# magicat777/Audio-Analyzer-OMEGA

Measured on NVIDIA B200. Metric: stream-seconds of 48 kHz stereo analysed/sec (multi-res FFT+LUFS+TP), higher is better.
Workload: dtype f32 (FFT, combine, K-weighting in a float32 delta-form state, sample peaks of the true-peak meter; its four transforms per frame pair in f16x2; tensor-core GEMM on (hi, lo) half operands with fp32 accumulators for the few-bin resolutions) + f64 (meter statistics)

## Files before the change

### audio-analyzer-omega_b200/csrc/kweight32_kernel.cuh

```cuda
#pragma once
#include <cuda_runtime.h>
#include "kweight_kernel.cuh"
#include "blockdft_tc_kernel.cuh"

namespace o4 {

struct Kw32Sec {
    float b0, a2, gamma, bb;
    float phi[5][4];
    float c16[4], c17[4];
    float g[KW_SUBMAX][2];
    float2 ga0[16], ga1[16];
};

struct Kweight32Args {
    const float* x;
    long long ch_stride, frame_stride, frame_off0;
    int n_ch, n_frames, first_frame, frames_per_warp;
    const float* hann;
    double* lufs_out;
    int rms_gate, _align;
    float* hop_inv;
    int hop_inv_nb, hop_inv_j0;
    Kw32Sec s[2];
};

__device__ __forceinline__ float2 kw32_mat(const float* m, float2 s) {
    return make_float2(fmaf(m[0], s.x, m[1] * s.y), fmaf(m[2], s.x, m[3] * s.y));
}

struct Kw32R { float r0; float2 a[16]; float2 b[16]; };

__device__ __forceinline__ float& kwr(Kw32R& q, int i) {
    if (i == 0) return q.r0;
    if (i <= 16) return q.a[i - 1].x;
    if (i <= 32) return q.b[i - 17].x;
    if (i <= 48) return q.b[i - 33].y;
    return q.a[i - 49].y;
}
__device__ __forceinline__ float2 bc2(float v) { return make_float2(v, v); }

template <bool BACKWARD>
__device__ __forceinline__ void kw32_pass(Kw32R& q, const Kw32Sec& c, int lane) {
    const int pos = BACKWARD ? 31 - lane : lane;
    const float b0 = c.b0, a2 = c.a2, ngamma = -c.gamma, bb = c.bb;
    float xa_in, dxa_in;
    {
        const float p1 = BACKWARD ? __shfl_down_sync(0xffffffffu, kwr(q, 0), 1) : __shfl_up_sync(0xffffffffu, kwr(q, KW_L - 1), 1);
        const float p2 = BACKWARD ? __shfl_down_sync(0xffffffffu, kwr(q, 1), 1) : __shfl_up_sync(0xffffffffu, kwr(q, KW_L - 2), 1);
        const float x0 = BACKWARD ? kwr(q, KW_L - 1) : kwr(q, 0);
        xa_in = pos == 0 ? x0 : p1;
        dxa_in = pos == 0 ? 0.f : p1 - p2;
    }
    const float2 s0 = make_float2(-b0 * xa_in, 0.f);
    float2 xaA, dxaA, xaB, dxaB;
    if (!BACKWARD) {
        xaA = make_float2(xa_in, kwr(q, 48)); dxaA = make_float2(dxa_in, kwr(q, 48) - kwr(q, 47));
        xaB = make_float2(kwr(q, 16), kwr(q, 32)); dxaB = make_float2(kwr(q, 16) - kwr(q, 15), kwr(q, 32) - kwr(q, 31));
    } else {
        xaA = make_float2(kwr(q, 17), xa_in); dxaA = make_float2(kwr(q, 17) - kwr(q, 18), dxa_in);
        xaB = make_float2(kwr(q, 33), kwr(q, 49)); dxaB = make_float2(kwr(q, 33) - kwr(q, 34), kwr(q, 49) - kwr(q, 50));
    }
    float2 zA = bc2(0.f), dA = bc2(0.f), yA = make_float2(b0 * xaA.x, b0 * xaA.y);
    float2 zB = bc2(0.f), dB = bc2(0.f), yB = make_float2(b0 * xaB.x, b0 * xaB.y);
    if (!BACKWARD) {
        const float x = q.r0;
        const float t = fmaf(a2, dA.x, dxaA.x);
        const float d = fmaf(ngamma, yA.x, t);
        const float z = fmaf(bb, d, zA.x);
        const float y = fmaf(b0, x, z);
        dxaA.x = x - xaA.x; xaA.x = x; zA.x = z; dA.x = d; yA.x = y;
        q.r0 = y;
    }
    const float2 A2 = bc2(a2), NG = bc2(ngamma), BB = bc2(bb), B0 = bc2(b0);
#pragma unroll
    for (int n = 0; n < 16; ++n) {
        const int k = BACKWARD ? 15 - n : n;
        {
            const float2 x = q.a[k];
            const float2 t = __ffma2_rn(A2, dA, dxaA);
            const float2 d = __ffma2_rn(NG, yA, t);
            const float2 z = __ffma2_rn(BB, d, zA);
            const float2 y = __ffma2_rn(B0, x, z);
            dxaA = __fadd2_rn(x, make_float2(-xaA.x, -xaA.y)); xaA = x; zA = z; dA = d; yA = y;
            q.a[k] = y;
        }
        {
            const float2 x = q.b[k];
            const float2 t = __ffma2_rn(A2, dB, dxaB);
            const float2 d = __ffma2_rn(NG, yB, t);
            const float2 z = __ffma2_rn(BB, d, zB);
            const float2 y = __ffma2_rn(B0, x, z);
            dxaB = __fadd2_rn(x, make_float2(-xaB.x, -xaB.y)); xaB = x; zB = z; dB = d; yB = y;
            q.b[k] = y;
        }
    }
    if (BACKWARD) {
        const float x = q.r0;
        const float t = fmaf(a2, dA.x, dxaA.x);
        const float d = fmaf(ngamma, yA.x, t);
        const float z = fmaf(bb, d, zA.x);
        const float y = fmaf(b0, x, z);
        zA.x = z; dA.x = d;
        q.r0 = y;
    }
    float2 e[KW_NSUB];
    if (!BACKWARD) { e[0] = make_float2(zA.x, dA.x); e[1] = make_float2(zB.x, dB.x); e[2] = make_float2(zB.y, dB.y); e[3] = make_float2(zA.y, dA.y); }
    else           { e[0] = make_float2(zA.y, dA.y); e[1] = make_float2(zB.y, dB.y); e[2] = make_float2(zB.x, dB.x); e[3] = make_float2(zA.x, dA.x); }
    float2 v = e[0];
#pragma unroll
    for (int m = 1; m < KW_NSUB; ++m) {
        const int j = BACKWARD ? KW_NSUB - 1 - m : m;
        const float* cm = (kw_off(j + 1) - kw_off(j) == 17) ? c.c17 : c.c16;
        const float2 w = kw32_mat(cm, v);
        v = make_float2(w.x + e[m].x, w.y + e[m].y);
    }
    if (pos == 0) {
        const float2 w = kw32_mat(c.phi[0], s0);
        v.x += w.x; v.y += w.y;
    }
#pragma unroll
    for (int jj = 0; jj < 5; ++jj) {
        const int dd = 1 << jj;
        const float rx = BACKWARD ? __shfl_down_sync(0xffffffffu, v.x, dd) : __shfl_up_sync(0xffffffffu, v.x, dd);
        const float ry = BACKWARD ? __shfl_down_sync(0xffffffffu, v.y, dd) : __shfl_up_sync(0xffffffffu, v.y, dd);
        if (pos >= dd) {
            const float2 w = kw32_mat(c.phi[jj], make_float2(rx, ry));
            v.x += w.x; v.y += w.y;
        }
    }
    float2 sin[KW_NSUB];
    sin[0].x = BACKWARD ? __shfl_down_sync(0xffffffffu, v.x, 1) : __shfl_up_sync(0xffffffffu, v.x, 1);
    sin[0].y = BACKWARD ? __shfl_down_sync(0xffffffffu, v.y, 1) : __shfl_up_sync(0xffffffffu, v.y, 1);
    if (pos == 0) sin[0] = s0;
#pragma unroll
    for (int m = 1; m < KW_NSUB; ++m) {
        const int jp = BACKWARD ? KW_NSUB - m : m - 1;
        const float* cm = (kw_off(jp + 1) - kw_off(jp) == 17) ? c.c17 : c.c16;
        const float2 w = kw32_mat(cm, sin[m - 1]);
        sin[m] = make_float2(w.x + e[m - 1].x, w.y + e[m - 1].y);
    }
    const float2 s_c0 = BACKWARD ? sin[3] : sin[0], s_c1 = BACKWARD ? sin[2] : sin[1];
    const float2 s_c2 = BACKWARD ? sin[1] : sin[2], s_c3 = BACKWARD ? sin[0] : sin[3];
    const float2 SXA = make_float2(s_c0.x, s_c3.x), SYA = make_float2(s_c0.y, s_c3.y);
    const float2 SXB = make_float2(s_c1.x, s_c2.x), SYB = make_float2(s_c1.y, s_c2.y);
    if (!BACKWARD) {
        q.r0 = fmaf(c.g[0][0], s_c0.x, fmaf(c.g[0][1], s_c0.y, q.r0));
#pragma unroll
        for (int k = 0; k < 16; ++k) {
            q.a[k] = __ffma2_rn(c.ga0[k], SXA, __ffma2_rn(c.ga1[k], SYA, q.a[k]));
            q.b[k] = __ffma2_rn(bc2(c.g[k][0]), SXB, __ffma2_rn(bc2(c.g[k][1]), SYB, q.b[k]));
        }
    } else {
#pragma unroll
        for (int k = 0; k < 16; ++k) {
            const float2 G0 = bc2(c.g[15 - k][0]), G1 = bc2(c.g[15 - k][1]);
            q.a[k] = __ffma2_rn(G0, SXA, __ffma2_rn(G1, SYA, q.a[k]));
            q.b[k] = __ffma2_rn(G0, SXB, __ffma2_rn(G1, SYB, q.b[k]));
        }
        q.r0 = fmaf(c.g[16][0], s_c0.x, fmaf(c.g[16][1], s_c0.y, q.r0));
    }
}

__device__ __forceinline__ void kw32_odd_pad(Kw32R& q, int lane) {
    if (lane == 0) {
#pragma unroll
        for (int j = 0; j < KW_PAD; ++j) kwr(q, j) = 2.f * kwr(q, KW_PAD) - kwr(q, 2 * KW_PAD - j);
    }
    if (lane == 31) {
        constexpr int E = KW_LAST - KW_PAD;
#pragma unroll
        for (int j = 0; j < KW_PAD; ++j) kwr(q, E + 1 + j) = 2.f * kwr(q, E) - kwr(q, E - 1 - j);
#pragma unroll
        for (int i = KW_LAST + 1; i < KW_L; ++i) kwr(q, i) = kwr(q, KW_LAST);
    }
}

__device__ __forceinline__ void kw32_fill_slack(Kw32R& q, int lane) {
    if (lane == 31) {
#pragma unroll
        for (int i = KW_LAST + 1; i < KW_L; ++i) kwr(q, i) = kwr(q, KW_LAST);
    }
}

__device__ __forceinline__ void kw32_zero_pads(Kw32R& q, int lane) {
    if (lane == 0) {
#pragma unroll
        for (int i = 0; i < KW_PAD; ++i) kwr(q, i) = 0.f;
    }
    if (lane == 31) {
#pragma unroll
        for (int i = KW_LAST - KW_PAD + 1; i < KW_L; ++i) kwr(q, i) = 0.f;
    }
}

constexpr int KW32_WARPS = 4;
#ifndef KW32_MIN_BLOCKS
#define KW32_MIN_BLOCKS 3
#endif

__global__ void __launch_bounds__(KW32_WARPS * 32, KW32_MIN_BLOCKS)
kweight32_kernel(const __grid_constant__ Kweight32Args a) {
    extern __shared__ __align__(16) unsigned char smem_raw[];
    float* hann_x = reinterpret_cast<float*>(smem_raw);
    float* stage_all = hann_x + 32 * KW_L;
    const int lane = threadIdx.x & 31;
    const int warp = threadIdx.x >> 5;
    float* stg = stage_all + warp * KW_STG;

    for (int p = threadIdx.x; p < 32 * KW_L; p += blockDim.x) {
        const int n = p - KW_PAD;
        hann_x[p] = (n >= 0 && n < KW_W) ? a.hann[n] : 0.f;
    }
    __syncthreads();

    const int frames_per_cta = a.frames_per_warp * KW32_WARPS;
    const int tiles_per_ch = (a.n_frames + frames_per_cta - 1) / frames_per_cta;
    const int ch = blockIdx.x / tiles_per_ch;
    const int tile = blockIdx.x % tiles_per_ch;

    for (int it = 0; it < a.frames_per_warp; ++it) {
        const int f = tile * frames_per_cta + it * KW32_WARPS + warp;
        if (f >= a.n_frames || f < a.first_frame) continue;
        const long long off = (long long)ch * a.ch_stride + a.frame_off0 + (long long)f * a.frame_stride;

        const float4* px = reinterpret_cast<const float4*>(a.x + off);
        float4* s4 = reinterpret_cast<float4*>(stg + KW_PAD + KW_STG_SHIFT);
        float4 tmp[KW_W / 4 / 32];
#pragma unroll
        for (int j = 0; j < KW_W / 4 / 32; ++j) tmp[j] = __ldg(px + lane + 32 * j);
        if (a.hop_inv) {
            float m = 0.f;
#pragma unroll
            for (int j = 3 * KW_W / 4 / 4 / 32; j < KW_W / 4 / 32; ++j)
                m = fmaxf(fmaxf(m, fmaxf(fabsf(tmp[j].x), fabsf(tmp[j].y))), fmaxf(fabsf(tmp[j].z), fabsf(tmp[j].w)));
#pragma unroll
            for (int o = 16; o > 0; o >>= 1) m = fmaxf(m, __shfl_xor_sync(0xffffffffu, m, o));
            if (lane == 0) a.hop_inv[(size_t)ch * a.hop_inv_nb + (f - a.hop_inv_j0)] = hop_row_scale(m);
        }
        if (lane < KW_PAD) stg[KW_STG_SHIFT + lane] = 0.f;
        if (lane < KW_SLACK + KW_PAD + KW_STG_SHIFT) stg[KW_STG_SHIFT + KW_PAD + KW_W + lane] = 0.f;
#pragma unroll
        for (int j = 0; j < KW_W / 4 / 32; ++j) s4[lane + 32 * j] = tmp[j];
        __syncwarp();
        float* sl = stg + KW_STG_SHIFT + KW_L * lane;
        const float* hl = hann_x + KW_L * lane;
        Kw32R r;
        float sumsq = 0.f;
#pragma unroll
        for (int i = 0; i < KW_L; ++i) {
            const float xv = sl[i] * hl[i];
            sumsq = fmaf(xv, xv, sumsq);
            kwr(r, i) = xv;
        }
        __syncwarp();
#pragma unroll
        for (int o = 16; o > 0; o >>= 1) sumsq += __shfl_xor_sync(0xffffffffu, sumsq, o);
        const bool gated = a.rms_gate && sqrtf(sumsq * (1.f / KW_W)) < 1e-6f;

        double ms = 0.0;
        if (!gated) {
#ifdef KW32_UNROLL_SECTIONS
#pragma unroll
#else
#pragma unroll 1
#endif
            for (int si = 0; si < 2; ++si) {
                const Kw32Sec& c = a.s[si];
                kw32_odd_pad(r, lane);
                kw32_pass<false>(r, c, lane);
                kw32_fill_slack(r, lane);
                kw32_pass<true>(r, c, lane);
                if (si == 0) {
                    kw32_zero_pads(r, lane);
#pragma unroll
                    for (int i = 0; i < KW_L; ++i) sl[i] = kwr(r, i);
                }
            }
            kw32_zero_pads(r, lane);
            float acc = 0.f;
#pragma unroll
            for (int i = 0; i < KW_L; ++i) {
                const float fv = sl[i];
                const float w = fmaf(kwr(r, i) - fv, 0.3f, fv);
                acc = fmaf(w, w, acc);
            }
#pragma unroll
            for (int o = 16; o > 0; o >>= 1) acc += __shfl_xor_sync(0xffffffffu, acc, o);
            ms = (double)acc / (double)KW_W;
            __syncwarp();
        }
        if (lane == 0)
            a.lufs_out[(size_t)ch * a.n_frames + f] = (ms > 1e-10) ? (-0.691 + 10.0 * log10(ms)) : -100.0;
    }
}

inline size_t kweight32_smem_bytes() {
    return (size_t)32 * KW_L * sizeof(float) + (size_t)KW32_WARPS * KW_STG * sizeof(float);
}

}
```

### audio-analyzer-omega_b200/csrc/omega4_cuda.cu

```cuda
#include "../../include/omega4_cuda.h"

#include <cuda_runtime.h>
#include <math.h>
#include <stdio.h>
#include <stdlib.h>
#include <string.h>

#include <algorithm>
#include <map>
#include <mutex>
#include <set>
#include <string>
#include <vector>

#include "bars_kernel.cuh"
#include "blockdft_kernel.cuh"
#include "blockdft_tc_kernel.cuh"
#include "fft_core.cuh"
#include "kweight_kernel.cuh"
#include "kweight32_kernel.cuh"
#include "loudness_kernel.cuh"
#include "misc_kernels.cuh"
#include "octave_kernel.cuh"
#include "multires_kernel.cuh"
// ... 155 lines not shown

static int launch_kweight(const KweightArgs& a, cudaStream_t s) {
    if (a.x_is_f64) return a.weighted_out ? launch_kweight_t<true, true>(a, s) : launch_kweight_t<true, false>(a, s);
    return a.weighted_out ? launch_kweight_t<false, true>(a, s) : launch_kweight_t<false, false>(a, s);
}

static int launch_kweight32(const Kweight32Args& a, cudaStream_t s) {
    const size_t smem = kweight32_smem_bytes();
    CK(cudaFuncSetAttribute(kweight32_kernel, cudaFuncAttributeMaxDynamicSharedMemorySize, (int)smem));
    const int fpc = a.frames_per_warp * KW32_WARPS;
    const long long grid = (long long)((a.n_frames + fpc - 1) / fpc) * a.n_ch;
    if (grid <= 0) return OMEGA4_OK;
    if (grid > 2147483647LL) return fail(OMEGA4_ERR_INVALID, "kweight grid too large");
    kweight32_kernel<<<(unsigned)grid, KW32_WARPS * 32, smem, s>>>(a);
    CK(cudaGetLastError());
    return OMEGA4_OK;
}

static int launch_stats(const StatsArgs& a, cudaStream_t s) {
    if (a.n_ch <= 0) return OMEGA4_OK;
    if (!a.fresh && a.n_frames == 1 && a.first_frame == 0 && !getenv("OMEGA4_STATS_WALK")) {
        stats_push1_kernel<<<a.n_ch, ST_P1_THREADS, 0, s>>>(a);
    } else if (a.fresh) {
        const size_t smem = stats_smem_bytes<false>();
        CK(cudaFuncSetAttribute(stats_kernel<false>, cudaFuncAttributeMaxDynamicSharedMemorySize, (int)smem));
        stats_kernel<false><<<a.n_ch, ST_THREADS, smem, s>>>(a);
    } else {
        const size_t smem = stats_smem_bytes<true>();
        CK(cudaFuncSetAttribute(stats_kernel<true>, cudaFuncAttributeMaxDynamicSharedMemorySize, (int)smem));
        stats_kernel<true><<<a.n_ch, ST_THREADS, smem, s>>>(a);
    }
    CK(cudaGetLastError());
    return OMEGA4_OK;
}

static int launch_s16_convert(const int16_t* in, long long stream_stride, int il, int n_streams, long long n_frames,
                              float* out, long long out_stride, cudaStream_t s) {
    if (n_streams <= 0 || n_frames <= 0) return OMEGA4_OK;
    if (n_streams > 65535) return fail(OMEGA4_ERR_INVALID, "too many streams for one int16 conversion launch (max 65535)");
    const long long per_stream = n_frames * il;
    dim3 grid((unsigned)((per_stream + 1023) / 1024), (unsigned)n_streams);
    s16_deinterleave_kernel<<<grid, 256, 0, s>>>(in, stream_stride, il, n_frames, out, out_stride);
    CK(cudaGetLastError());
    return OMEGA4_OK;
}

static void mat2_mul(const double* a, const double* b, double* c) {
    double r[4] = {a[0] * b[0] + a[1] * b[2], a[0] * b[1] + a[1] * b[3],
                   a[2] * b[0] + a[3] * b[2], a[2] * b[1] + a[3] * b[3]};
    memcpy(c, r, sizeof r);
}

static void build_biquad(const double* b, const double* a, int order, KwBiquad* q) {
    memset(q, 0, sizeof *q);
    const double a0 = a[0];
    q->b0 = b[0] / a0; q->b1 = b[1] / a0; q->b2 = order >= 2 ? b[2] / a0 : 0.0;
    q->a1 = a[1] / a0; q->a2 = order >= 2 ? a[2] / a0 : 0.0;
    q->pad = 3 * (order + 1);
    if (order >= 2) {
        double zi0, zi1;
        const double m00 = 1.0 + q->a1, m01 = -1.0, m10 = q->a2, m11 = 1.0;
        const double r0 = q->b1 - q->a1 * q->b0, r1 = q->b2 - q->a2 * q->b0;
        const double det = m00 * m11 - m01 * m10;
        zi0 = (r0 * m11 - m01 * r1) / det;
        zi1 = (m00 * r1 - m10 * r0) / det;
        q->yi0 = -zi1 / q->a2;
        q->yi1 = (-zi0 + q->a1 * zi1 / q->a2) / q->a2;
    } else {
        const double zi0 = (q->b1 - q->a1 * q->b0) / (1.0 + q->a1);
        q->yi0 = -zi0 / q->a1;
        q->yi1 = 0.0;
    }
    const double Cm[4] = {-q->a1, -q->a2, 1.0, 0.0};
    double P[4] = {Cm[0], Cm[1], Cm[2], Cm[3]};
    for (int i = 0; i < KW_L; ++i) {
        if (i < KW_SUBMAX) { q->g[i][0] = P[0]; q->g[i][1] = P[1]; }
        if (i + 1 == 16) memcpy(q->c16, P, sizeof P);
        if (i + 1 == 17) memcpy(q->c17, P, sizeof P);
        if (i + 1 < KW_L) mat2_mul(Cm, P, P);
    }
    memcpy(q->phi[0], P, sizeof P);
    for (int j = 1; j < 5; ++j) mat2_mul(q->phi[j - 1], q->phi[j - 1], q->phi[j]);
    auto inv_pow = [&](int k, double* out) {
        if (k == 0) { out[0] = 1; out[1] = 0; out[2] = 0; out[3] = 1; return; }
        if (order >= 2) {
            const double det1 = Cm[0] * Cm[3] - Cm[1] * Cm[2];
            const double Ci[4] = {Cm[3] / det1, -Cm[1] / det1, -Cm[2] / det1, Cm[0] / det1};
            double R[4] = {Ci[0], Ci[1], Ci[2], Ci[3]};
            for (int i = 1; i < k; ++i) mat2_mul(Ci, R, R);
            memcpy(out, R, sizeof R);
        } else {
            out[0] = pow(-q->a1, -(double)k); out[1] = 0; out[2] = 0; out[3] = 0;
        }
    };
    inv_pow(KW_PAD - q->pad, q->cinv_f);
    inv_pow(KW_SLACK + KW_PAD - q->pad, q->cinv_b);
}

struct ResInfo {
    int n = 0, log2m = 0, bins = 0;
    float weight = 1.f;
    float* window = nullptr;
    float* binw = nullptr;
    int n_tb = 0;
    int* tb_idx = nullptr;
    int* tb_lo = nullptr;
    float* tb_frac = nullptr;
    int need_lo = 0, need_cnt = 0;
    Twiddles tw;
};

struct SparseRes {
    int r = 0, nk = 0, nt = 0, B = 0, col0 = 0;
    bool td = false;
    int xoff = 0;
    float2* T = nullptr;
    float* kw = nullptr;
    int* tb_pos = nullptr;
};

struct SparseSet {
    int n = 0;
    SparseRes sp[OMEGA4_MAX_RES];
    int of_res[OMEGA4_MAX_RES];
    int cols = 0, qs = 0;
    float* E = nullptr;
    uint8_t* Eimg = nullptr;
    float e_inv = 1.f;
    int n_halves = 0;
    bool fusable = false;
    int nkx = 0;
    short gB[TC_MAX_GROUPS], gX[TC_MAX_GROUPS], gN[TC_MAX_GROUPS], gS[TC_MAX_GROUPS];
    SparseSet() { for (int i = 0; i < OMEGA4_MAX_RES; ++i) of_res[i] = -1; }
    void release() {
        for (int i = 0; i < OMEGA4_MAX_RES; ++i) { cudaFree(sp[i].T); cudaFree(sp[i].kw); cudaFree(sp[i].tb_pos); }
        cudaFree(E); cudaFree(Eimg);
    }
};

struct DevBuf {
    void* p = nullptr;
    size_t cap = 0;
    int ensure(size_t bytes) {
        if (bytes <= cap) return OMEGA4_OK;
        if (p) cudaFree(p);
        p = nullptr; cap = 0;
        CK(cudaMalloc(&p, bytes));
        cap = bytes;
        return OMEGA4_OK;
    }
    void release() { if (p) cudaFree(p); p = nullptr; cap = 0; }
};

struct omega4_bars {
    int device = 0, T = 0, n_valid = 0, p_lo = 0, normalize_max = 0;
    float p_frac = 0.f, scale = 0.8f;
    int* bands = nullptr; float* gain = nullptr; float* sf = nullptr; float* sfc = nullptr;
    DevBuf h_spec, h_out, h_peak, h_state, state_in;
};

static int bars_launch(omega4_bars* b, cudaStream_t s, const float* spec, int n_ch, int n_hops, float* state, int fresh,
                       float* band_values, float* peak_values, DevBuf* state_copy) {
    BarsArgs a;
    memset(&a, 0, sizeof a);
    a.T = b->T; a.n_ch = n_ch; a.n_hops = n_hops; a.n_valid = b->n_valid; a.bands = b->bands; a.gain = b->gain;
    a.sf = b->sf; a.sfc = b->sfc; a.p_lo = b->p_lo; a.p_frac = b->p_frac; a.scale = b->scale;
    a.normalize_max = b->normalize_max; a.fresh = (fresh || !state) ? 1 : 0;
    a.spec = spec; a.bars_out = band_values; a.peaks_out = peak_values; a.state = state;
    const size_t st_bytes = (size_t)n_ch * (1 + b->n_valid) * sizeof(float);
    const size_t smem = bars_smem_bytes(b->T, b->n_valid);
    if (smem > 200 * 1024) return fail(OMEGA4_ERR_UNSUPPORTED, "spectrum too long for the bars kernel");
    if (b->T > 32 * BARS_MAXV) return fail(OMEGA4_ERR_UNSUPPORTED, "spectrum too long for the bars kernel (max 1024 bins)");
    if (b->T <= 512) CK(cudaFuncSetAttribute(bars_kernel<16>, cudaFuncAttributeMaxDynamicSharedMemorySize, (int)smem));
    else CK(cudaFuncSetAttribute(bars_kernel<32>, cudaFuncAttributeMaxDynamicSharedMemorySize, (int)smem));
    a.seg = n_ch >= 1024 ? 4 * BARS_SEG : BARS_SEG;
    const long long grid = (long long)n_ch * ((n_hops + a.seg - 1) / a.seg);
    if (grid > 2147483647LL) return fail(OMEGA4_ERR_INVALID, "bars grid too large");
    if (a.state && !a.fresh && n_hops > a.seg) {
        int rc = state_copy->ensure(st_bytes); if (rc) return rc;
        CK(cudaMemcpyAsync(state_copy->p, a.state, st_bytes, cudaMemcpyDeviceToDevice, s));
        a.state_in = (const float*)state_copy->p;
    }
    if (b->T <= 512) bars_kernel<16><<<(unsigned)grid, BARS_WARPS * 32, smem, s>>>(a);
    else bars_kernel<32><<<(unsigned)grid, BARS_WARPS * 32, smem, s>>>(a);
    CK(cudaGetLastError());
    return OMEGA4_OK;
}

struct BarsReq {
    omega4_bars* b = nullptr;
    float* band_values = nullptr; float* peak_values = nullptr; float* state = nullptr;
    int fresh = 1;
};

struct KernelTime { char name[32]; cudaEvent_t e0, e1; };

struct SideCtx {
    cudaStream_t side = nullptr;
    cudaEvent_t ev_fork = nullptr, ev_tp = nullptr, ev_join = nullptr;
    int ensure() {
        if (side) return OMEGA4_OK;
        CK(cudaStreamCreateWithFlags(&side, cudaStreamNonBlocking));
        CK(cudaEventCreateWithFlags(&ev_fork, cudaEventDisableTiming));
        CK(cudaEventCreateWithFlags(&ev_tp, cudaEventDisableTiming));
        CK(cudaEventCreateWithFlags(&ev_join, cudaEventDisableTiming));
        return OMEGA4_OK;
    }
    void release() {
        if (side) cudaStreamDestroy(side);
        if (ev_fork) cudaEventDestroy(ev_fork);
        if (ev_tp) cudaEventDestroy(ev_tp);
        if (ev_join) cudaEventDestroy(ev_join);
        side = nullptr; ev_fork = ev_tp = ev_join = nullptr;
    }
};

struct omega4_plan {
    int device = 0;
    int sample_rate = 48000, hop = 512, n_res = 0, T = 0, W = OMEGA4_METER_WINDOW;
    double gate = -70.0;
    ResInfo res[OMEGA4_MAX_RES];
    bool disjoint = true;
    int* csr_ptr = nullptr; int* csr_res = nullptr; int* csr_lo = nullptr; float* csr_frac = nullptr;
    double* hann64 = nullptr;
    float* hann32 = nullptr;
    KwBiquad kw_default[2];
    KwBiquad kw[4];
    int kw_nsec = 2, kw_blend = 1, kw_gate = 1;
    double kw_gain = 1.0;
    Twiddles tw_meter;
    float2* tp_rot = nullptr;
    unsigned* tp_rot_h = nullptr;
    SparseSet set_cc;
    SparseSet set_tc;
    bool tensor_default = true;
    DevBuf scratch_lufs, scratch_tp, scratch_mag[OMEGA4_MAX_RES], scratch_q, scratch_f32, scratch_comb, scratch_bstate, scratch_inv;
    DevBuf h_in, h_comb, h_meters, h_state, h_mag[OMEGA4_MAX_RES], h_f64a, h_f64b, h_f64c;
    struct Slot {
        cudaStream_t s = nullptr;
        DevBuf in, in16, comb, met, lufs, tp, state, q, mag[OMEGA4_MAX_RES];
        DevBuf bars, peaks, bstate, bstate_copy;
        SideCtx sc;
    };
#ifndef OMEGA4_HOST_SLOTS
#define OMEGA4_HOST_SLOTS 4
#endif
    static constexpr int N_SLOTS = OMEGA4_HOST_SLOTS;
    Slot slots[N_SLOTS];
    size_t host_chunk_bytes = (size_t)1024 << 20;
    SideCtx sc;
    long long launches = 0;
    std::vector<KernelTime> times;
    size_t n_times = 0;
};

static void set_weighting_k(omega4_plan* p) {
    p->kw[0] = p->kw_default[0]; p->kw[1] = p->kw_default[1];
    p->kw_nsec = 2; p->kw_blend = 1; p->kw_gate = 1; p->kw_gain = 1.0;
}

static double max_pole_radius(const KwBiquad& q) {
    if (q.a2 == 0.0) return fabs(q.a1);
    const double disc = q.a1 * q.a1 - 4.0 * q.a2;
    if (disc < 0.0) return sqrt(q.a2);
    return fmax(fabs(-q.a1 + sqrt(disc)), fabs(-q.a1 - sqrt(disc))) * 0.5;
}

static void to_float(const KwBiquad& s, KwBiquadF* d) {
    d->b0 = (float)s.b0; d->b1 = (float)s.b1; d->b2 = (float)s.b2; d->a1 = (float)s.a1; d->a2 = (float)s.a2;
    d->yi0 = (float)s.yi0; d->yi1 = (float)s.yi1; d->pad = s.pad; d->_align = 0;
    for (int j = 0; j < 5; ++j) for (int e = 0; e < 4; ++e) d->phi[j][e] = (float)s.phi[j][e];
    for (int e = 0; e < 4; ++e) {
        d->cinv_f[e] = (float)s.cinv_f[e]; d->cinv_b[e] = (float)s.cinv_b[e];
        d->c16[e] = (float)s.c16[e]; d->c17[e] = (float)s.c17[e];
    }
    for (int i = 0; i < KW_SUBMAX; ++i) { d->g[i][0] = (float)s.g[i][0]; d->g[i][1] = (float)s.g[i][1]; }
}

static bool is_highpass_biquad(const KwBiquad& q) {
    return q.pad == 9 && q.a2 != 0.0 && fabs(q.b1 + 2.0 * q.b0) <= 1e-12 * fabs(q.b0) && fabs(q.b2 - q.b0) <= 1e-12 * fabs(q.b0);
}

static void build_kw32(const KwBiquad& q, Kw32Sec* o) {
    const double alpha = 1.0 + q.a1 + q.a2, beta = 1.0 - q.a2;
    const double bb = -q.b0 * beta, gamma = alpha / bb;
    o->b0 = (float)q.b0; o->a2 = (float)q.a2; o->gamma = (float)gamma; o->bb = (float)bb;
    const double M[4] = {1.0 - alpha, bb * q.a2, -gamma, q.a2};
    double P[4] = {M[0], M[1], M[2], M[3]};
    for (int i = 0; i < KW_L; ++i) {
        if (i < KW_SUBMAX) { o->g[i][0] = (float)P[0]; o->g[i][1] = (float)P[1]; }
        if (i + 1 == 16) for (int e = 0; e < 4; ++e) o->c16[e] = (float)P[e];
        if (i + 1 == 17) for (int e = 0; e < 4; ++e) o->c17[e] = (float)P[e];
        if (i + 1 < KW_L) mat2_mul(M, P, P);
    }
    for (int k = 0; k < 16; ++k) {
        o->ga0[k] = make_float2(o->g[k + 1][0], o->g[k][0]);
        o->ga1[k] = make_float2(o->g[k + 1][1], o->g[k][1]);
    }
    double Q[4] = {P[0], P[1], P[2], P[3]};
    for (int j = 0; j < 5; ++j) {
        for (int e = 0; e < 4; ++e) o->phi[j][e] = (float)Q[e];
        mat2_mul(Q, Q, Q);
    }
}

static bool use_kweight32(const omega4_plan* p) {
    return p->W == KW_W && p->kw_nsec == 2 && p->kw_blend && p->kw_gain == 1.0 && is_highpass_biquad(p->kw[0]) &&
           is_highpass_biquad(p->kw[1]) && !getenv("OMEGA4_KW_F64");
}

static void fill_weighting(const omega4_plan* p, KweightArgs* k) {
    k->n_sec = p->kw_nsec; k->blend = p->kw_blend; k->rms_gate = p->kw_gate; k->gain = p->kw_gain;
    for (int i = 0; i < p->kw_nsec; ++i) { k->f[i] = p->kw[i]; to_float(p->kw[i], &k->ff[i]); }
    int from = p->kw_nsec;
    while (from > 1 && max_pole_radius(p->kw[from - 1]) < 0.95) --from;
    k->f32_from = getenv("OMEGA4_KW_F64") ? p->kw_nsec : from;
}

static int upload(void** dst, const void* src, size_t bytes) {
    CK(cudaMalloc(dst, bytes ? bytes : 1));
    if (bytes) CK(cudaMemcpy(*dst, src, bytes, cudaMemcpyHostToDevice));
    return OMEGA4_OK;
}

static size_t boff_of(const omega4_plan_desc* d, int r) {
    size_t o = 0;
    for (int i = 0; i < r; ++i) o += (size_t)d->fft_sizes[i] / 2 + 1;
    return o;
}

static int build_sparse_set(omega4_plan* p, const omega4_plan_desc* d, const std::vector<std::vector<int>>& idx,
                            const std::vector<std::vector<int>>& lo, bool tensor, SparseSet* set) {
    const int H = d->hop;
    if ((H % (tensor ? TC_KC : BD_KC)) != 0) return OMEGA4_OK;
    const int max_cols = tensor ? TC_MAX_GROUPS * 32 : 128;
    const bool allow_td = tensor && !getenv("OMEGA4_BLOCKDFT_FD");
    int order[OMEGA4_MAX_RES];
    for (int r = 0; r < d->n_res; ++r) order[r] = r;
    for (int i = 0; i < d->n_res; ++i)
        for (int j = i + 1; j < d->n_res; ++j)
            if (p->res[order[j]].n > p->res[order[i]].n) { int t = order[i]; order[i] = order[j]; order[j] = t; }
    std::vector<std::vector<float>> ecols;
    int cols = 0;
    size_t woff2[OMEGA4_MAX_RES];
    { size_t o = 0; for (int r = 0; r < d->n_res; ++r) { woff2[r] = o; o += d->fft_sizes[r]; } }
    for (int oi = 0; oi < d->n_res; ++oi) {
        const int r = order[oi];
        const ResInfo& ri = p->res[r];
        const int N = ri.n;
        if (N % H != 0 || N / H < 2 || N / H > 64) continue;
        std::vector<int> bins;
        for (int l : lo[r]) if (l >= 0) { bins.push_back(l); bins.push_back(l + 1); }
        std::sort(bins.begin(), bins.end());
        bins.erase(std::unique(bins.begin(), bins.end()), bins.end());
        if (bins.empty()) continue;
        const float* w = d->windows + woff2[r];
        const double two_pi = 6.283185307179586476925287;
        const int nk = (int)bins.size();
        const double fft_cost = 2.5 * N * (ri.log2m + 1);
        if (allow_td && N / H <= 64 && (double)(2 * nk * (N / H)) * H <= 6.6 * fft_cost &&
            ((cols + 31) & ~31) + 2 * nk * (N / H) <= max_cols) {
            cols = (cols + 31) & ~31;
            SparseRes& sp = set->sp[set->n];
            sp.r = r; sp.nk = nk; sp.nt = N / H; sp.B = N / H; sp.col0 = cols; sp.td = true;
            const int rc_cols = 2 * nk * sp.B;
            std::vector<float> ec((size_t)H * rc_cols);
            std::vector<float> kw(nk);
            for (int ki = 0; ki < nk; ++ki) {
                kw[ki] = d->bin_weights ? d->bin_weights[boff_of(d, r) + bins[ki]] : 1.f;
                for (int b = 0; b < sp.B; ++b)
                    for (int n2 = 0; n2 < H; ++n2) {
                        const int i = H * b + n2;
                        const long long ph = ((long long)bins[ki] * i) % N;
                        const double ang = -two_pi * (double)ph / (double)N;
                        ec[(size_t)n2 * rc_cols + 2 * (ki * sp.B + b)] = (float)((double)w[i] * cos(ang));
                        ec[(size_t)n2 * rc_cols + 2 * (ki * sp.B + b) + 1] = (float)((double)w[i] * sin(ang));
                    }
            }
            std::vector<int> pos(idx[r].size(), -1);
            for (size_t j = 0; j < lo[r].size(); ++j)
                if (lo[r][j] >= 0) pos[j] = (int)(std::lower_bound(bins.begin(), bins.end(), lo[r][j]) - bins.begin());
            int rc = upload((void**)&sp.kw, kw.data(), kw.size() * sizeof(float)); if (rc) return rc;
            rc = upload((void**)&sp.tb_pos, pos.data(), pos.size() * sizeof(int)); if (rc) return rc;
            set->of_res[r] = set->n++;
            ecols.push_back(std::move(ec));
            cols += rc_cols;
            cols = (cols + 31) & ~31;
            continue;
        }
        const double phi = 6.283185307179586476925287 / (double)(N - 1);
        double G[3][4] = {{0}};
        for (int i = 0; i < N; ++i) {
            const double c[3] = {1.0, cos(phi * i), cos(2.0 * phi * i)};
            for (int u = 0; u < 3; ++u) { for (int v = 0; v < 3; ++v) G[u][v] += c[u] * c[v]; G[u][3] += c[u] * (double)w[i]; }
        }
        bool singular = false;
        for (int u = 0; u < 3 && !singular; ++u) {
            int piv = u;
            for (int v = u + 1; v < 3; ++v) if (fabs(G[v][u]) > fabs(G[piv][u])) piv = v;
            if (fabs(G[piv][u]) < 1e-9) { singular = true; break; }
            if (piv != u) for (int c2 = 0; c2 < 4; ++c2) { double t = G[u][c2]; G[u][c2] = G[piv][c2]; G[piv][c2] = t; }
            for (int v = 0; v < 3; ++v) {
                if (v == u) continue;
                const double f = G[v][u] / G[u][u];
                for (int c2 = 0; c2 < 4; ++c2) G[v][c2] -= f * G[u][c2];
            }
        }
        if (singular) continue;
        double am[3] = {G[0][3] / G[0][0], G[1][3] / G[1][1], G[2][3] / G[2][2]};
        double resid = 0.0;
        for (int i = 0; i < N; ++i) {
            const double fit = am[0] + am[1] * cos(phi * i) + am[2] * cos(2.0 * phi * i);
            resid = fmax(resid, fabs(fit - (double)w[i]));
        }
        if (resid > 1.5e-7) continue;
        int tm[5]; double tc[5]; int nt = 0;
        tm[nt] = 0; tc[nt] = am[0]; ++nt;
        for (int m = 1; m <= 2; ++m)
            if (fabs(am[m]) > 1e-9) { tm[nt] = m; tc[nt] = 0.5 * am[m]; ++nt; tm[nt] = -m; tc[nt] = 0.5 * am[m]; ++nt; }
        const int rc_cols = 2 * nk * nt;
        if (!tensor && (double)rc_cols * H * 2.0 > fft_cost) continue;
        if (tensor && (double)rc_cols * H > 6.6 * fft_cost) continue;
        if (cols + rc_cols > max_cols) continue;
        SparseRes& sp = set->sp[set->n];
        sp.r = r; sp.nk = nk; sp.nt = nt; sp.B = N / H; sp.col0 = cols;
        std::vector<float> ec((size_t)H * rc_cols);
        std::vector<float2> T((size_t)nk * sp.B * nt);
        std::vector<float> kw(nk);
        for (int ki = 0; ki < nk; ++ki) {
            kw[ki] = d->bin_weights ? d->bin_weights[boff_of(d, r) + bins[ki]] : 1.f;
            for (int t = 0; t < nt; ++t) {
                const double th = tm[t] * phi - two_pi * (double)bins[ki] / (double)N;
                for (int n2 = 0; n2 < H; ++n2) {
                    const double ang = fmod(th * n2, two_pi);
                    ec[(size_t)n2 * rc_cols + 2 * (ki * nt + t)] = (float)cos(ang);
                    ec[(size_t)n2 * rc_cols + 2 * (ki * nt + t) + 1] = (float)sin(ang);
                }
                for (int b = 0; b < sp.B; ++b) {
                    const double ang = fmod(th * (double)H * b, two_pi);
                    T[((size_t)ki * sp.B + b) * nt + t] = make_float2((float)(tc[t] * cos(ang)), (float)(tc[t] * sin(ang)));
                }
            }
        }
        std::vector<int> pos(idx[r].size(), -1);
        for (size_t j = 0; j < lo[r].size(); ++j)
            if (lo[r][j] >= 0) pos[j] = (int)(std::lower_bound(bins.begin(), bins.end(), lo[r][j]) - bins.begin());
        int rc = upload((void**)&sp.T, T.data(), T.size() * sizeof(float2)); if (rc) return rc;
        rc = upload((void**)&sp.kw, kw.data(), kw.size() * sizeof(float)); if (rc) return rc;
        rc = upload((void**)&sp.tb_pos, pos.data(), pos.size() * sizeof(int)); if (rc) return rc;
        set->of_res[r] = set->n++;
        ecols.push_back(std::move(ec));
        cols += rc_cols;
    }
    if (set->n == 0) return OMEGA4_OK;
    set->cols = cols;
    if (!tensor) {
        set->qs = cols <= 32 ? 32 : (cols <= 64 ? 64 : 128);
        std::vector<float> E((size_t)H * set->qs, 0.f);
        for (int si = 0; si < set->n; ++si) {
            const SparseRes& sp = set->sp[si];
            const int rc_cols = 2 * sp.nk * sp.nt;
            for (int n2 = 0; n2 < H; ++n2)
                memcpy(&E[(size_t)n2 * set->qs + sp.col0], &ecols[si][(size_t)n2 * rc_cols], rc_cols * sizeof(float));
        }
        return upload((void**)&set->E, E.data(), E.size() * sizeof(float));
    }
    set->n_halves = (cols + TC_BN - 1) / TC_BN;
    set->qs = set->n_halves * TC_BN;
    {
        bool ok = set->n_halves * (TC_BN / 32) <= TC_MAX_GROUPS;
        int xo = 0;
        for (int si = 0; si < set->n; ++si) {
            SparseRes& sp = set->sp[si];
            ok = ok && sp.td && (sp.B == 2 || sp.B == 4 || sp.B == 8 || sp.B == 16 || sp.B == 32 || sp.B == 64) && (sp.col0 % 32) == 0;
            sp.xoff = xo; xo += sp.nk;
        }
        set->nkx = xo;
        for (int g = 0; g < TC_MAX_GROUPS; ++g) { set->gB[g] = 0; set->gX[g] = 0; set->gN[g] = 0; set->gS[g] = -1; }
        if (ok)
            for (int si = 0; si < set->n; ++si) {
                const SparseRes& sp = set->sp[si];
                if (sp.B > 16) {
                    const int parts = sp.B / 16;
                    for (int k0 = 0; k0 < sp.nk; ++k0)
                        for (int pt = 0; pt < parts; ++pt) {
                            const int g = (sp.col0 + 2 * (k0 * sp.B + 16 * pt)) / 32;
                            set->gB[g] = 16; set->gX[g] = (short)(sp.xoff + k0); set->gN[g] = 1;
                            set->gS[g] = (short)(sp.B - 16 * (pt + 1));
                        }
                    continue;
                }
                const int per = 16 / sp.B;
                for (int k0 = 0; k0 < sp.nk; k0 += per) {
                    const int g = (sp.col0 + 2 * k0 * sp.B) / 32;
                    set->gB[g] = (short)sp.B; set->gX[g] = (short)(sp.xoff + k0);
                    set->gN[g] = (short)((sp.nk - k0 < per) ? sp.nk - k0 : per);
                }
            }
        set->fusable = ok && !getenv("OMEGA4_BLOCKDFT_UNFUSED");
    }
    const int nkc = H / TC_KC;
    std::vector<uint8_t> img((size_t)set->n_halves * nkc * 2 * TC_B_BYTES, 0);
#if TC_F16
    float emax = 0.f;
    for (const auto& ec : ecols) for (float v : ec) emax = fmaxf(emax, fabsf(v));
    int eexp = 0;
    if (emax > 0.f) frexpf(emax, &eexp);
    const float escale = ldexpf(1.f, -eexp);
    set->e_inv = ldexpf(1.f, eexp);
#endif
    for (int si = 0; si < set->n; ++si) {
        const SparseRes& sp = set->sp[si];
        const int rc_cols = 2 * sp.nk * sp.nt;
        for (int cc = 0; cc < rc_cols; ++cc) {
            const int col = sp.col0 + cc, h = col / TC_BN, n = col % TC_BN;
            for (int k = 0; k < H; ++k) {
                const float v = ecols[si][(size_t)k * rc_cols + cc];
#if TC_F16
                const float vs = v * escale;
                const __half hh = __float2half_rn(vs);
                const __half hl = __float2half_rn((vs - __half2float(hh)) * TC_LO_SCALE);
                const int kc = k / TC_KC, e = k % TC_KC;
                const size_t base = ((size_t)(h * nkc + kc) * 2) * TC_B_BYTES;
                const int off = tc_sw64_offset(n, e >> 3) + (e & 7) * 2;
                memcpy(&img[base + off], &hh, 2);
                memcpy(&img[base + TC_B_BYTES + off], &hl, 2);
#else
                uint32_t bits; memcpy(&bits, &v, 4); bits &= 0xFFFFE000u;
                float hi; memcpy(&hi, &bits, 4);
                const float lo2 = v - hi;
                const int kc = k / TC_KC, e = k % TC_KC;
                const size_t base = ((size_t)(h * nkc + kc) * 2) * TC_B_BYTES;
                const int off = tc_sw64_offset(n, e >> 2) + (e & 3) * 4;
                memcpy(&img[base + off], &hi, 4);
                memcpy(&img[base + TC_B_BYTES + off], &lo2, 4);
#endif
            }
        }
    }
    return upload((void**)&set->Eimg, img.data(), img.size());
}

static int plan_build(omega4_plan* p, const omega4_plan_desc* d) {
    if (d->n_res < 1 || d->n_res > OMEGA4_MAX_RES) return fail(OMEGA4_ERR_INVALID, "n_res must be 1..8");
    if (d->hop <= 0 || (d->hop % 4) != 0) return fail(OMEGA4_ERR_INVALID, "hop must be a positive multiple of 4");
    if (d->target_bins < 1) return fail(OMEGA4_ERR_INVALID, "target_bins must be >= 1");
    if (d->meter_window != OMEGA4_METER_WINDOW) return fail(OMEGA4_ERR_UNSUPPORTED, "meter_window must be 2048");
    if (!d->fft_sizes || !d->windows || !d->tb_count || !d->res_weight || !d->meter_hann || !d->kw_coeffs)
        return fail(OMEGA4_ERR_INVALID, "plan_desc has NULL tables");
    p->sample_rate = d->sample_rate; p->hop = d->hop; p->n_res = d->n_res; p->T = d->target_bins;
    p->gate = d->gate_threshold;
    std::vector<int> owners(d->target_bins, 0);
    size_t woff = 0, boff = 0, toff = 0;
    std::vector<std::vector<int>> idx(d->n_res), lo(d->n_res);
    std::vector<std::vector<float>> fr(d->n_res);
    for (int r = 0; r < d->n_res; ++r) {
        ResInfo& ri = p->res[r];
        const int n = d->fft_sizes[r];
        if (!is_pow2(n) || n < 512 || n > 32768) return fail(OMEGA4_ERR_UNSUPPORTED, "fft size must be a power of two in 512 .. 32768");
        ri.n = n; ri.log2m = ilog2(n) - 1; ri.bins = n / 2 + 1; ri.weight = d->res_weight[r];
        if (ri.weight <= 0.f) return fail(OMEGA4_ERR_INVALID, "resolution weight must be positive");
        int rc = upload((void**)&ri.window, d->windows + woff, (size_t)n * sizeof(float));
        if (rc) return rc;
        if (d->bin_weights) { rc = upload((void**)&ri.binw, d->bin_weights + boff, (size_t)ri.bins * sizeof(float)); if (rc) return rc; }
        woff += n; boff += ri.bins;
        const int cnt = d->tb_count[r];
        if (cnt < 0) return fail(OMEGA4_ERR_INVALID, "negative tb_count");
        for (int j = 0; j < cnt; ++j) {
            const int ti = d->tb_idx[toff + j], l = d->tb_lo[toff + j];
            if (ti < 0 || ti >= d->target_bins || l < 0 || l + 1 >= ri.bins)
                return fail(OMEGA4_ERR_INVALID, "combine table entry out of range");
            idx[r].push_back(ti); lo[r].push_back(l); fr[r].push_back(d->tb_frac[toff + j]);
            owners[ti]++;
        }
        toff += cnt;
        rc = get_twiddles(p->device, ri.log2m, &ri.tw);
        if (rc) return rc;
    }
    p->disjoint = true;
    for (int t = 0; t < d->target_bins; ++t) if (owners[t] > 1) p->disjoint = false;
    {
        std::vector<int> ptr(d->target_bins + 1, 0), cres, clo;
        std::vector<float> cfr;
        for (int t = 0; t < d->target_bins; ++t) {
            for (int r = 0; r < d->n_res; ++r)
                for (size_t j = 0; j < idx[r].size(); ++j)
                    if (idx[r][j] == t) { cres.push_back(r); clo.push_back(lo[r][j]); cfr.push_back(fr[r][j]); }
            ptr[t + 1] = (int)cres.size();
        }
        int rc = upload((void**)&p->csr_ptr, ptr.data(), ptr.size() * sizeof(int)); if (rc) return rc;
        rc = upload((void**)&p->csr_res, cres.data(), cres.size() * sizeof(int)); if (rc) return rc;
        rc = upload((void**)&p->csr_lo, clo.data(), clo.size() * sizeof(int)); if (rc) return rc;
        rc = upload((void**)&p->csr_frac, cfr.data(), cfr.size() * sizeof(float)); if (rc) return rc;
    }
    for (int r = 0; r < d->n_res; ++r) {
        ResInfo& ri = p->res[r];
        int mn = 1 << 30, mx = -1;
        for (int l : lo[r]) { if (l < mn) mn = l; if (l > mx) mx = l; }
        if (mx >= 0) { ri.need_lo = mn; ri.need_cnt = mx + 2 - mn; } else { ri.need_lo = 0; ri.need_cnt = 0; }
        if (r == 0)
            for (int t = 0; t < d->target_bins; ++t)
                if (owners[t] == 0) { idx[0].push_back(t); lo[0].push_back(-1); fr[0].push_back(0.f); }
        ri.n_tb = (int)idx[r].size();
        int rc = upload((void**)&ri.tb_idx, idx[r].data(), idx[r].size() * sizeof(int)); if (rc) return rc;
        rc = upload((void**)&ri.tb_lo, lo[r].data(), lo[r].size() * sizeof(int)); if (rc) return rc;
        rc = upload((void**)&ri.tb_frac, fr[r].data(), fr[r].size() * sizeof(float)); if (rc) return rc;
// ... 1547 lines not shown
```

Baseline: 283,900.

## Truncate K-weight scan by pole decay and fuse Hann windowing into staging

The host computes a per-section scan depth from the pole radius raised to the chunk length, and the warp-level prefix scan stops early once the carried state has decayed below 2^-30. Hann windowing and the sum of squares are now fused into the global-to-shared staging using packed float2 multiplies, so the padded per-lane Hann table in shared memory is no longer needed and shared memory use drops. The first-section output is stored in a conflict-free float2 layout and blended with packed FMA before the energy sum. Skipping scan steps assumes the decay bound holds, which introduces a small approximation in the filter state.

New measurement: 284,000, median of 6. Within noise of the previous version (+0.0%).

```diff
diff --git a/audio-analyzer-omega_b200/csrc/kweight32_kernel.cuh b/audio-analyzer-omega_b200/csrc/kweight32_kernel.cuh
--- a/audio-analyzer-omega_b200/csrc/kweight32_kernel.cuh
+++ b/audio-analyzer-omega_b200/csrc/kweight32_kernel.cuh
@@ -11,6 +11,8 @@
     float c16[4], c17[4];
     float g[KW_SUBMAX][2];
     float2 ga0[16], ga1[16];
+    int depth;
+    int _align;
 };
 
 struct Kweight32Args {
@@ -121,6 +123,7 @@
     }
 #pragma unroll
     for (int jj = 0; jj < 5; ++jj) {
+        if (jj == c.depth) break;
         const int dd = 1 << jj;
         const float rx = BACKWARD ? __shfl_down_sync(0xffffffffu, v.x, dd) : __shfl_up_sync(0xffffffffu, v.x, dd);
         const float ry = BACKWARD ? __shfl_down_sync(0xffffffffu, v.y, dd) : __shfl_up_sync(0xffffffffu, v.y, dd);
@@ -202,16 +205,14 @@
 __global__ void __launch_bounds__(KW32_WARPS * 32, KW32_MIN_BLOCKS)
 kweight32_kernel(const __grid_constant__ Kweight32Args a) {
     extern __shared__ __align__(16) unsigned char smem_raw[];
-    float* hann_x = reinterpret_cast<float*>(smem_raw);
-    float* stage_all = hann_x + 32 * KW_L;
+    float4* hann4 = reinterpret_cast<float4*>(smem_raw);
+    float* stage_all = reinterpret_cast<float*>(hann4 + KW_W / 4);
     const int lane = threadIdx.x & 31;
     const int warp = threadIdx.x >> 5;
     float* stg = stage_all + warp * KW_STG;
-
-    for (int p = threadIdx.x; p < 32 * KW_L; p += blockDim.x) {
-        const int n = p - KW_PAD;
-        hann_x[p] = (n >= 0 && n < KW_W) ? a.hann[n] : 0.f;
-    }
+    float2* st2 = reinterpret_cast<float2*>(stg);
+
+    for (int p = threadIdx.x; p < KW_W / 4; p += blockDim.x) hann4[p] = reinterpret_cast<const float4*>(a.hann)[p];
     __syncthreads();
 
     const int frames_per_cta = a.frames_per_warp * KW32_WARPS;
@@ -240,20 +241,22 @@
         }
         if (lane < KW_PAD) stg[KW_STG_SHIFT + lane] = 0.f;
         if (lane < KW_SLACK + KW_PAD + KW_STG_SHIFT) stg[KW_STG_SHIFT + KW_PAD + KW_W + lane] = 0.f;
-#pragma unroll
-        for (int j = 0; j < KW_W / 4 / 32; ++j) s4[lane + 32 * j] = tmp[j];
+        float2 sq = bc2(0.f);
+#pragma unroll
+        for (int j = 0; j < KW_W / 4 / 32; ++j) {
+            const float4 h = hann4[lane + 32 * j];
+            const float2 lo = __fmul2_rn(make_float2(tmp[j].x, tmp[j].y), make_float2(h.x, h.y));
+            const float2 hi = __fmul2_rn(make_float2(tmp[j].z, tmp[j].w), make_float2(h.z, h.w));
+            sq = __ffma2_rn(hi, hi, __ffma2_rn(lo, lo, sq));
+            s4[lane + 32 * j] = make_float4(lo.x, lo.y, hi.x, hi.y);
+        }
         __syncwarp();
-        float* sl = stg + KW_STG_SHIFT + KW_L * lane;
-        const float* hl = hann_x + KW_L * lane;
+        const float* sl = stg + KW_STG_SHIFT + KW_L * lane;
         Kw32R r;
-        float sumsq = 0.f;
-#pragma unroll
-        for (int i = 0; i < KW_L; ++i) {
-            const float xv = sl[i] * hl[i];
-            sumsq = fmaf(xv, xv, sumsq);
-            kwr(r, i) = xv;
-        }
+#pragma unroll
+        for (int i = 0; i < KW_L; ++i) kwr(r, i) = sl[i];
         __syncwarp();
+        float sumsq = sq.x + sq.y;
 #pragma unroll
         for (int o = 16; o > 0; o >>= 1) sumsq += __shfl_xor_sync(0xffffffffu, sumsq, o);
         const bool gated = a.rms_gate && sqrtf(sumsq * (1.f / KW_W)) < 1e-6f;
@@ -274,17 +277,25 @@
                 if (si == 0) {
                     kw32_zero_pads(r, lane);
 #pragma unroll
-                    for (int i = 0; i < KW_L; ++i) sl[i] = kwr(r, i);
+                    for (int k = 0; k < 16; ++k) { st2[32 * k + lane] = r.a[k]; st2[32 * (16 + k) + lane] = r.b[k]; }
+                    stg[2048 + lane] = r.r0;
                 }
             }
             kw32_zero_pads(r, lane);
+            {
+                const float2 C = bc2(0.3f);
+                const float f0 = stg[2048 + lane];
+                r.r0 = fmaf(r.r0 - f0, 0.3f, f0);
+#pragma unroll
+                for (int k = 0; k < 16; ++k) {
+                    const float2 fa = st2[32 * k + lane], fb = st2[32 * (16 + k) + lane];
+                    r.a[k] = __ffma2_rn(__fadd2_rn(r.a[k], make_float2(-fa.x, -fa.y)), C, fa);
+                    r.b[k] = __ffma2_rn(__fadd2_rn(r.b[k], make_float2(-fb.x, -fb.y)), C, fb);
+                }
+            }
             float acc = 0.f;
 #pragma unroll
-            for (int i = 0; i < KW_L; ++i) {
-                const float fv = sl[i];
-                const float w = fmaf(kwr(r, i) - fv, 0.3f, fv);
-                acc = fmaf(w, w, acc);
-            }
+            for (int i = 0; i < KW_L; ++i) acc = fmaf(kwr(r, i), kwr(r, i), acc);
 #pragma unroll
             for (int o = 16; o > 0; o >>= 1) acc += __shfl_xor_sync(0xffffffffu, acc, o);
             ms = (double)acc / (double)KW_W;
@@ -296,7 +307,7 @@
 }
 
 inline size_t kweight32_smem_bytes() {
-    return (size_t)32 * KW_L * sizeof(float) + (size_t)KW32_WARPS * KW_STG * sizeof(float);
-}
-
-}
+    return (size_t)KW_W * sizeof(float) + (size_t)KW32_WARPS * KW_STG * sizeof(float);
+}
+
+}
diff --git a/audio-analyzer-omega_b200/csrc/omega4_cuda.cu b/audio-analyzer-omega_b200/csrc/omega4_cuda.cu
--- a/audio-analyzer-omega_b200/csrc/omega4_cuda.cu
+++ b/audio-analyzer-omega_b200/csrc/omega4_cuda.cu
@@ -481,6 +481,10 @@
         for (int e = 0; e < 4; ++e) o->phi[j][e] = (float)Q[e];
         mat2_mul(Q, Q, Q);
     }
+    const double r65 = pow(max_pole_radius(q), (double)KW_L);
+    o->depth = 5;
+    for (int d = 1; d < 5; ++d)
+        if (pow(r65, (double)(1 << d)) < 0x1p-30) { o->depth = d; break; }
 }
 
 static bool use_kweight32(const omega4_plan* p) {
```
